# liudabao001/JABD-Joint-Attention-Based-Detector-for-small-face-detection

Hardware: AMD Instinct MI355X
Metric: images/sec at 1024x1024 bs32 (1/2/4/8 GPU); boxes/sec NMS (higher is better)
Workload: dtype fp32; 1 GPU; C2: JABD-MobileNetV3 RetinaFace (nets/retinaface_r.py) eval forward, weights_init weights; global_batch=32, image_size=1024, parallelism=replicas x1

## Files before the change

include/jabd.h:

```cpp
#ifndef JABD_H_
#define JABD_H_

#include <stddef.h>
#include <stdint.h>

#ifdef __cplusplus
extern "C" {
#endif

typedef void* jabd_stream_t;

enum {
  JABD_OK = 0,
  JABD_EINVAL = 1,
  JABD_EHIP = 2,
  JABD_EWS = 3,
};

const char* jabd_version(void);
int64_t jabd_abi_struct_size(int32_t which);
int jabd_last_error(char* buf, size_t len);

int jabd_decode_f32(const float* loc, const float* priors, int64_t batch,
                    int64_t num_priors, float var0, float var1, float* boxes,
// ... 113 lines not shown
                               const int64_t* counts,
                               float* grad_loc, float* grad_conf,
                               float* grad_landm, jabd_stream_t stream);
int jabd_multibox_diou_loss_fwd_f32(const float* loc, const float* conf,
                                    const float* landm, const float* loc_t,
                                    const int64_t* conf_t, const float* landm_t,
                                    const float* priors, float var0, float var1,
                                    int64_t batch, int64_t num_priors, int neg_pos,
                                    float* sums, int64_t* counts, uint8_t* sel,
                                    void* ws, size_t ws_bytes, jabd_stream_t stream);
int jabd_multibox_diou_loss_bwd_f32(const float* loc, const float* conf,
                                    const float* landm, const float* loc_t,
                                    const int64_t* conf_t, const float* landm_t,
                                    const float* priors, float var0, float var1,
                                    const uint8_t* sel, int64_t batch,
                                    int64_t num_priors, const float* gout,
                                    const int64_t* counts, float* grad_loc,
                                    float* grad_conf, float* grad_landm,
                                    jabd_stream_t stream);
int jabd_multibox_loss_finalize_f32(const float* sums, const int64_t* counts,
                                    float* loss, jabd_stream_t stream);

enum {
  JABD_ACT_NONE = 0,
  JABD_ACT_RELU = 1,
  JABD_ACT_LEAKY = 2,
  JABD_ACT_HSWISH = 3,
  JABD_ACT_HSIGMOID = 4,
  JABD_ACT_SIGMOID = 5,
};

typedef struct jabd_conv_args {
  const float* x; int64_t x_bs; int32_t x_ps, x_c0;
  int32_t B, H, W, Cin;
  const float* x2; int64_t x2_bs; int32_t x2_ps, Cin2;
  int32_t x2_W, x2_stride;
  const float* ascale; int64_t ascale_bs;
  const void* w; const float* bias;
  const float* res; int64_t res_bs; int32_t res_ps, res_c0;
  float* y; int64_t y_bs; int32_t y_ps, y_c0;
  int32_t OH, OW, Cout, Ntiles, tn, Kc;
  int32_t KH, KW, stride, pad;
  int32_t act; float slope;
  int32_t nchw_in, tconv;
  int32_t flags, reserved1;
  int64_t M;
  const void* w32; int32_t ntiles32, tn32;
  float* y2; int64_t y2_bs; int32_t y2_ps, y2_c0, nsplit, act2; float slope2; int32_t reserved2;
  void* ws; int64_t ws_bytes;
} jabd_conv_args;
int64_t jabd_conv_workspace_size(const jabd_conv_args* args);
int jabd_conv_pack_tn(int cout);
int jabd_conv_pack_tn32(int cout);
int jabd_conv_pack_f32(const float* w, int32_t cout, int32_t cin, int32_t kh, int32_t kw,
                       int32_t transposed, int32_t Kc, int32_t Ntiles, float* wp, int32_t K8,
                       int32_t NT32, float* wp32, jabd_stream_t stream);
int jabd_conv_pack_multi_f32(const int64_t* jobs, const int64_t* starts, int32_t njobs,
                             int64_t total, jabd_stream_t stream);
int jabd_conv2d_nhwc_f32(const jabd_conv_args* args, jabd_stream_t stream);
int64_t jabd_conv1x1_bn_stats_nblk(const jabd_conv_args* args);
int64_t jabd_conv_bn_bwd_part_floats(const jabd_conv_args* args);
int jabd_conv_bn_bwd_sums_f32(const jabd_conv_args* args, const float* x, int32_t x_ps,
                              const float* mean, const float* invstd, const float* gamma,
                              const float* beta, int32_t act, float slope, float* part,
                              int64_t part_floats, jabd_stream_t stream);
int jabd_conv_bn_bwd_sums_res_f32(const jabd_conv_args* args, const float* x, int32_t x_ps,
                                  const float* mask, int32_t mask_ps, const float* mean,
                                  const float* invstd, float* part, int64_t part_floats,
                                  jabd_stream_t stream);
int jabd_bn_act_bwd_rows_f32(float* part, const float* dy, const float* x, int64_t M,
                             int32_t C, const float* mean, const float* invstd,
                             const float* gamma, const float* beta, int32_t act, float slope,
                             float* dgamma, float* dbeta, float* dx, jabd_stream_t stream);
int64_t jabd_conv_bn_stats_part_floats(const jabd_conv_args* args);
int jabd_conv_bn_stats_f32(const jabd_conv_args* args, float* part, int64_t part_floats,
                           float* mean, float* invstd, float* running_mean, float* running_var,
                           float momentum, float eps, jabd_stream_t stream);
int jabd_conv1x1_bn_stats_f32(const jabd_conv_args* args, float* part, int64_t nblk,
                              float* shift, jabd_stream_t stream);

int jabd_stem_nchw_f32(const float* x, int32_t B, int32_t H, int32_t W, const float* w,
                       const float* bias, int32_t act, float* y, jabd_stream_t stream);

typedef struct jabd_dw_args {
  const float* x; int64_t x_bs; int32_t x_ps, reserved0;
  int32_t B, H, W, C;
  const float* w; const float* bias;
  float* y; int64_t y_bs; int32_t y_ps, reserved1;
  int32_t OH, OW, k, stride, pad, act;
  float slope; int32_t nblk;
  float* part;
} jabd_dw_args;
int64_t jabd_dw_nblk(int64_t B, int64_t OH, int64_t OW, int64_t C);
int jabd_dwconv_nhwc_f32(const jabd_dw_args* args, jabd_stream_t stream);
int64_t jabd_dwconv_stats_nblk(int64_t B, int64_t OH, int64_t OW, int64_t C);
int jabd_dwconv_stats_f32(const jabd_dw_args* args, float* stats_part, float* shift,
                          jabd_stream_t stream);
int jabd_dwconv_bnin_stats_f32(const jabd_dw_args* args, const float* mean, const float* invstd,
                               const float* gamma, const float* beta, int32_t act, float slope,
                               float* stats_part, float* shift, jabd_stream_t stream);

typedef struct jabd_expdw_args {
  const float* x; int64_t x_bs; int32_t x_ps, Cin;
  int32_t B, H, W, E;
  const void* we; const float* be; int32_t Ntiles, Kc;
  const float* wd; const float* bd;
// ... 200 lines not shown
```

jabd-joint-attention-based-detector-for-small-face-detection_amd/csrc/conv32.hip:

```cpp
#include <stdlib.h>

#include <algorithm>

#include "common.h"
#include "conv_args.h"

namespace jabd {

typedef float f32x16 __attribute__((ext_vector_type(16)));

__device__ __forceinline__ float act32(float v, int act, float slope) {
  switch (act) {
    case ACT_RELU: return relu_f(v);
    case ACT_LEAKY: return v > 0.f ? v : v * slope;
    case ACT_HSWISH: return hswish_f(v);
    case ACT_HSIGMOID: return hsigmoid_f(v);
    case ACT_SIGMOID: return 1.f / (1.f + expf(-v));
    default: return v;
  }
}

constexpr int kBK = 32;

__device__ __forceinline__ void wave_lds_sync32() {
  asm volatile("s_waitcnt lgkmcnt(0)" ::: "memory");
  __builtin_amdgcn_wave_barrier();
}
constexpr int kG = kBK / 8;
constexpr int kGateLds = 1024;

constexpr int kEpiPitch = 36;
enum { kEpiRt = 0, kEpiNone = 1, kEpiRes = 2 };
template <int TN, bool ST, bool BB, int EPI = kEpiRt>
__device__ __forceinline__ void m32_epilogue_tm1(const ConvArgs& p, const f32x16 (&acc)[TN],
                                                 int pm, int om, int nb, int srow, float* ep,
                                                 float* __restrict__ part, const BnEpi& bb,
                                                 int lane) {
  const bool has_bias = EPI == kEpiRt && p.bias;
  const bool has_res = EPI == kEpiRes || (EPI == kEpiRt && p.res);
  const int h = lane >> 5, j = lane & 31;
  const int ep_px = lane >> 3, ep_q = lane & 7;
  int mrow[4], prow[4];
#pragma unroll
  for (int r = 0; r < 4; ++r) {
    prow[r] = __shfl(pm, ep_px + 8 * r);
    mrow[r] = __shfl(om, ep_px + 8 * r);
  }
#pragma unroll
  for (int u = 0; u < TN; ++u) {
    const int nb0 = (nb * TN + u) * 32;
    if (nb0 >= p.Cout) break;
    const int n = nb0 + 4 * ep_q;
    float4 ss = make_float4(0.f, 0.f, 0.f, 0.f), sq = ss, sh = ss;
    float4 bmu = sh, bis = sh, bgm = sh, bbt = sh;
    float4 bx[4], bmk[4];
    if constexpr (BB) {
      if (n < p.Cout) {
        bmu = *reinterpret_cast<const float4*>(bb.mean + n);
        bis = *reinterpret_cast<const float4*>(bb.invstd + n);
        if (!bb.mask) {
          bgm = *reinterpret_cast<const float4*>(bb.gamma + n);
          bbt = *reinterpret_cast<const float4*>(bb.beta + n);
        }
      }
#pragma unroll
      for (int r = 0; r < 4; ++r)
        bx[r] = (prow[r] >= 0 && n < p.Cout)
                    ? *reinterpret_cast<const float4*>(bb.x + (int64_t)mrow[r] * bb.x_ps + n)
                    : sh;
      if (bb.mask) {
#pragma unroll
        for (int r = 0; r < 4; ++r)
          bmk[r] = (prow[r] >= 0 && n < p.Cout)
                       ? *reinterpret_cast<const float4*>(bb.mask + (int64_t)mrow[r] * bb.mask_ps + n)
                       : sh;
      }
    }
#pragma unroll
    for (int c = 0; c < 4; ++c)
      *reinterpret_cast<float4*>(ep + j * kEpiPitch + 8 * c + 4 * h) =
          make_float4(acc[u][4 * c], acc[u][4 * c + 1], acc[u][4 * c + 2],
                      acc[u][4 * c + 3]);
    wave_lds_sync32();
    if constexpr (ST) sh = *reinterpret_cast<const float4*>(ep + 4 * ep_q);
#pragma unroll
    for (int r = 0; r < 4; ++r) {
      const int px = ep_px + 8 * r;
      if (prow[r] < 0 || n >= p.Cout) continue;
      float4 v = *reinterpret_cast<const float4*>(ep + px * kEpiPitch + 4 * ep_q);
      if (BB && bb.mask) {
        if (p.res) {
          const float4 rr = *reinterpret_cast<const float4*>(p.res + (int64_t)mrow[r] * p.res_ps +
                                                             p.res_c0 + n);
          v.x += rr.x; v.y += rr.y; v.z += rr.z; v.w += rr.w;
        }
        v.x *= bmk[r].x > 0.f ? 1.f : 0.f;
        v.y *= bmk[r].y > 0.f ? 1.f : 0.f;
        v.z *= bmk[r].z > 0.f ? 1.f : 0.f;
        v.w *= bmk[r].w > 0.f ? 1.f : 0.f;
        const float xh0 = (bx[r].x - bmu.x) * bis.x, xh1 = (bx[r].y - bmu.y) * bis.y;
        const float xh2 = (bx[r].z - bmu.z) * bis.z, xh3 = (bx[r].w - bmu.w) * bis.w;
        ss.x += v.x; ss.y += v.y; ss.z += v.z; ss.w += v.w;
        sq.x += v.x * xh0; sq.y += v.y * xh1; sq.z += v.z * xh2; sq.w += v.w * xh3;
        *reinterpret_cast<float4*>(p.y + (int64_t)mrow[r] * p.y_ps + p.y_c0 + n) = v;
// ... 278 lines not shown
      for (int u = 0; u < TN; ++u) bw[u] = bs[(q * TN + u) * 64 + lane];
#pragma unroll
      for (int t = 0; t < TM; ++t)
#pragma unroll
        for (int u = 0; u < TN; ++u)
          acc[t][u] = __builtin_amdgcn_mfma_f32_32x32x2f32(bw[u].x, a_cur[t][q].x, acc[t][u], 0, 0, 0);
#pragma unroll
      for (int t = 0; t < TM; ++t)
#pragma unroll
        for (int u = 0; u < TN; ++u)
          acc[t][u] = __builtin_amdgcn_mfma_f32_32x32x2f32(bw[u].y, a_cur[t][q].y, acc[t][u], 0, 0, 0);
#pragma unroll
      for (int t = 0; t < TM; ++t)
#pragma unroll
        for (int u = 0; u < TN; ++u)
          acc[t][u] = __builtin_amdgcn_mfma_f32_32x32x2f32(bw[u].z, a_cur[t][q].z, acc[t][u], 0, 0, 0);
#pragma unroll
      for (int t = 0; t < TM; ++t)
#pragma unroll
        for (int u = 0; u < TN; ++u)
          acc[t][u] = __builtin_amdgcn_mfma_f32_32x32x2f32(bw[u].w, a_cur[t][q].w, acc[t][u], 0, 0, 0);
    }
    if (more) {
      store_b((s + 1) & 1, s + 1, b_nxt);
#pragma unroll
      for (int t = 0; t < TM; ++t)
#pragma unroll
        for (int q = 0; q < kG; ++q) a_cur[t][q] = a_nxt[t][q];
    }
    __syncthreads();
  }

  if (ks > 1) {
    const int npad = p.Ntiles * 32;
    float* pb = part + (int64_t)blockIdx.y * p.M * npad;
#pragma unroll
    for (int t = 0; t < TM; ++t) {
      if (pm[t] < 0) continue;
      float* prow = pb + (int64_t)om[t] * npad;
#pragma unroll
      for (int u = 0; u < TN; ++u)
#pragma unroll
        for (int c = 0; c < 4; ++c) {
          const int n = (nb * TN + u) * 32 + 8 * c + 4 * h;
          *reinterpret_cast<float4*>(prow + n) = make_float4(
              acc[t][u][4 * c], acc[t][u][4 * c + 1], acc[t][u][4 * c + 2], acc[t][u][4 * c + 3]);
        }
    }
    return;
  }
  if constexpr (TM == 1) {
    float* ep = reinterpret_cast<float*>(sB_) + wave * 32 * kEpiPitch;
    const int srow = mb * 4 + wave;
    m32_epilogue_tm1<TN, ST, BB, (ST || BB) ? kEpiNone : EPI>(p, acc[0], pm[0], om[0], nb, srow,
                                                                ep, part, bb, lane);
    return;
  }
#pragma unroll
  for (int t = 0; t < TM; ++t) {
    const int m = om[t];
    if (pm[t] < 0) continue;
    float* yrow = p.y + (int64_t)m * p.y_ps + p.y_c0;
    const float* rrow = p.res ? p.res + (int64_t)m * p.res_ps + p.res_c0 : nullptr;
#pragma unroll
    for (int u = 0; u < TN; ++u)
#pragma unroll
      for (int c = 0; c < 4; ++c) {
        const int n = (nb * TN + u) * 32 + 8 * c + 4 * h;
        if (n >= p.Cout) continue;
        float4 v = make_float4(acc[t][u][4 * c], acc[t][u][4 * c + 1], acc[t][u][4 * c + 2],
                               acc[t][u][4 * c + 3]);
        if (p.bias) {
          const float4 bb = *reinterpret_cast<const float4*>(p.bias + n);
          v.x += bb.x; v.y += bb.y; v.z += bb.z; v.w += bb.w;
        }
        if (rrow) {
          const float4 rr = *reinterpret_cast<const float4*>(rrow + n);
          v.x += rr.x; v.y += rr.y; v.z += rr.z; v.w += rr.w;
        }
        v.x = act32(v.x, p.act, p.slope);
        v.y = act32(v.y, p.act, p.slope);
        v.z = act32(v.z, p.act, p.slope);
        v.w = act32(v.w, p.act, p.slope);
        *reinterpret_cast<float4*>(yrow + n) = v;
      }
  }

}

__global__ __launch_bounds__(256) void m32_ksplit_reduce(const ConvArgs p, int ks,
                                                         const float* __restrict__ part) {
  const int npad = p.Ntiles * 32, c4n = (p.Cout + 3) >> 2;
  const int64_t i = blockIdx.x * (int64_t)blockDim.x + threadIdx.x;
  if (i >= p.M * c4n) return;
  const int64_t m = i / c4n;
  const int n = (int)(i - m * c4n) * 4;
  float4 v = *reinterpret_cast<const float4*>(part + m * npad + n);
  for (int y = 1; y < ks; ++y) {
    const float4 q = *reinterpret_cast<const float4*>(part + ((int64_t)y * p.M + m) * npad + n);
    v.x += q.x; v.y += q.y; v.z += q.z; v.w += q.w;
  }
  if (p.bias) {
    const float4 bb = *reinterpret_cast<const float4*>(p.bias + n);
    v.x += bb.x; v.y += bb.y; v.z += bb.z; v.w += bb.w;
  }
  if (p.res) {
    const float4 rr = *reinterpret_cast<const float4*>(p.res + m * p.res_ps + p.res_c0 + n);
    v.x += rr.x; v.y += rr.y; v.z += rr.z; v.w += rr.w;
  }
  v.x = act32(v.x, p.act, p.slope);
  v.y = act32(v.y, p.act, p.slope);
  v.z = act32(v.z, p.act, p.slope);
  v.w = act32(v.w, p.act, p.slope);
  *reinterpret_cast<float4*>(p.y + m * p.y_ps + p.y_c0 + n) = v;
}

template <int TN, int KS, bool ST, bool BB, int EPI>
__global__ __launch_bounds__(256) void conv1x1_m32s_kernel(const ConvArgs p, int nblk_n,
                                                            float* __restrict__ part,
                                                            const BnEpi bb) {
  constexpr int NW4 = KS * kG * TN * 64;
  extern __shared__ __attribute__((aligned(16))) float4 m32s_lds[];
  const int lane = threadIdx.x & 63;
  const int wave = __builtin_amdgcn_readfirstlane(threadIdx.x >> 6);
  const int h = lane >> 5, j = lane & 31;
  const int xcd = blockIdx.x & 7, rr = blockIdx.x >> 3;
  const int nb = rr % nblk_n, wgm = (rr / nblk_n) * 8 + xcd;
  const int gm = gridDim.x / nblk_n;
  {
    const float4* wg = reinterpret_cast<const float4*>(p.w);
    for (int f = threadIdx.x; f < NW4; f += 256) {
      const int k8 = f / (TN * 64), rem = f - k8 * (TN * 64);
      m32s_lds[f] = wg[((int64_t)k8 * p.Ntiles + nb * TN + (rem >> 6)) * 64 + (rem & 63)];
    }
  }
  __syncthreads();
  float* ep = reinterpret_cast<float*>(m32s_lds + NW4) + wave * 32 * kEpiPitch;
  const int64_t ntiles = (p.M + 31) >> 5;
  const int64_t step = (int64_t)gm * 4;
  const float* xb = p.x + p.x_c0 + 4 * h;
  auto load = [&](int64_t T, int s, int q) {
    const int64_t m = T * 32 + j;
    return m < p.M ? *reinterpret_cast<const float4*>(xb + m * p.x_ps + s * kBK + 8 * q)
                   : make_float4(0.f, 0.f, 0.f, 0.f);
  };
  float4 a[KS][kG];
  int64_t T = (int64_t)wgm * 4 + wave;
#pragma unroll
  for (int s = 0; s < KS; ++s)
#pragma unroll
    for (int q = 0; q < kG; ++q) a[s][q] = load(T, s, q);
  for (; T < ntiles; T += step) {
    const int64_t Tn = T + step;
    f32x16 acc[TN];
#pragma unroll
    for (int u = 0; u < TN; ++u)
#pragma unroll
      for (int r = 0; r < 16; ++r) acc[u][r] = 0.f;
#pragma unroll
    for (int s = 0; s < KS; ++s)
#pragma unroll
      for (int q = 0; q < kG; ++q) {
        float4 bw[TN];
#pragma unroll
        for (int u = 0; u < TN; ++u) bw[u] = m32s_lds[((s * kG + q) * TN + u) * 64 + lane];
#pragma unroll
        for (int u = 0; u < TN; ++u)
          acc[u] = __builtin_amdgcn_mfma_f32_32x32x2f32(bw[u].x, a[s][q].x, acc[u], 0, 0, 0);
#pragma unroll
        for (int u = 0; u < TN; ++u)
          acc[u] = __builtin_amdgcn_mfma_f32_32x32x2f32(bw[u].y, a[s][q].y, acc[u], 0, 0, 0);
#pragma unroll
        for (int u = 0; u < TN; ++u)
          acc[u] = __builtin_amdgcn_mfma_f32_32x32x2f32(bw[u].z, a[s][q].z, acc[u], 0, 0, 0);
#pragma unroll
        for (int u = 0; u < TN; ++u)
          acc[u] = __builtin_amdgcn_mfma_f32_32x32x2f32(bw[u].w, a[s][q].w, acc[u], 0, 0, 0);
        a[s][q] = load(Tn, s, q);
      }
    const int64_t m = T * 32 + j;
    const int pm = m < p.M ? (int)m : -1;
    m32_epilogue_tm1<TN, ST, BB, EPI>(p, acc, pm, pm, nb, (int)T, ep, part, bb, lane);
  }
}

static int m32_ksplit(const ConvArgs& a, bool kxk, int64_t grid) {
  if (a.tconv || a.Cout % 4 || grid >= 256) return 1;
  const int Kt = kxk ? a.KH * a.KW * a.Cin : a.Cin + (a.x2 ? a.Cin2 : 0);
  const int S = (Kt + kBK - 1) / kBK;
  int ks = (int)std::min<int64_t>(8, (512 + grid - 1) / grid);
  ks = std::min(ks, S / 4);
  return ks >= 2 ? ks : 1;
}
static int64_t m32_ksplit_bytes(const ConvArgs& a, int ks) {
  return ks > 1 ? (int64_t)ks * a.B * a.OH * a.OW * a.ntiles32 * 32 * (int64_t)sizeof(float) : 0;
}

template <int TM, int TN, bool KXK, bool AS>
static int launch_m32_as(const ConvArgs& a, hipStream_t st);

template <int TM, int TN, bool KXK>
static int launch_m32(const ConvArgs& a, hipStream_t st) {
  if (a.ascale) return launch_m32_as<TM, TN, KXK, true>(a, st);
  return launch_m32_as<TM, TN, KXK, false>(a, st);
}

template <int TM, int TN, bool KXK, bool AS>
static int launch_m32_as(const ConvArgs& a, hipStream_t st) {
  constexpr int BM = 4 * 32 * TM;
  const int64_t OHW = (int64_t)a.OH * a.OW;
  const int per_img = a.ascale != nullptr;
  const int64_t mt_img = cdiv(OHW, BM);
  if (KXK && a.tconv && a.stride == 2) {
    JABD_REQUIRE(!per_img, "conv32: phase mode without ascale");
    for (int ph = 0; ph < 2; ++ph)
      for (int pw = 0; pw < 2; ++pw) {
        const int64_t Mp = (int64_t)a.B * ((a.OH - ph + 1) / 2) * ((a.OW - pw + 1) / 2);
        if (Mp <= 0) continue;
        const int64_t grid = cdiv(Mp, BM) * (a.Ntiles / TN);
        JABD_REQUIRE(grid < (int64_t)0x7fffffff, "conv32: grid too large");
        conv1x1_m32_kernel<TM, TN, KXK, AS><<<(unsigned)grid, 256, 0, st>>>(a, (int)mt_img, 0,
                                                                        2 * ph + pw, 1, nullptr,
                                                                        BnEpi{});
        if (int e = check_launch("conv1x1_m32")) return e;
      }
    return JABD_OK;
  }
  const int64_t mtiles = per_img ? mt_img * a.B : cdiv(a.M, BM);
  const int64_t grid = mtiles * (a.Ntiles / TN);
  JABD_REQUIRE(grid < (int64_t)0x7fffffff, "conv32: grid too large");
  const int ks = a.ws ? m32_ksplit(a, KXK, grid) : 1;
  if (ks > 1 && a.ws_bytes >= m32_ksplit_bytes(a, ks)) {
    float* part = static_cast<float*>(a.ws);
    conv1x1_m32_kernel<TM, TN, KXK, AS><<<dim3((unsigned)grid, (unsigned)ks), 256, 0, st>>>(
        a, (int)mt_img, per_img, -1, ks, part, BnEpi{});
    if (int e = check_launch("conv1x1_m32 (split K)")) return e;
    const int64_t n4 = a.M * ((a.Cout + 3) / 4);
    m32_ksplit_reduce<<<(unsigned)cdiv(n4, 256), 256, 0, st>>>(a, ks, part);
    return check_launch("m32_ksplit_reduce");
  }
  if constexpr (TM == 1 && !AS) {
    if (!a.bias && a.act == ACT_NONE) {
      if (a.res)
        conv1x1_m32_kernel<1, TN, KXK, false, false, false, kEpiRes>
            <<<(unsigned)grid, 256, 0, st>>>(a, (int)mt_img, per_img, -1, 1, nullptr, BnEpi{});
      else
        conv1x1_m32_kernel<1, TN, KXK, false, false, false, kEpiNone>
            <<<(unsigned)grid, 256, 0, st>>>(a, (int)mt_img, per_img, -1, 1, nullptr, BnEpi{});
      return check_launch("conv1x1_m32");
    }
  }
  conv1x1_m32_kernel<TM, TN, KXK, AS><<<(unsigned)grid, 256, 0, st>>>(a, (int)mt_img, per_img, -1,
                                                                     1, nullptr, BnEpi{});
  return check_launch("conv1x1_m32");
}

static bool m32s_on() {
  static const bool on = [] {
    const char* e = getenv("JABD_M32S");
    return !(e && e[0] == '0');
  }();
  return on;
}

// ... 103 lines not shown
using namespace jabd;

static int m32_tm(const ConvArgs& a) {
  static int ftm = -1;
  if (ftm < 0) {
    const char* e = getenv("JABD_M32_TM");
    ftm = e ? atoi(e) : 0;
  }
  if (a.tn32 > 4) return 1;
  if (ftm == 1 || ftm == 2) return ftm;
  return (!a.ascale || a.M < 65536) ? 1 : 2;
}

static int m32_tn_launch(const ConvArgs& a) {
  static const bool off = [] {
    const char* e = getenv("JABD_M32_TN1");
    return e && e[0] == '0';
  }();
  if (off || a.tn32 <= 1 || a.tconv || !a.ascale) return a.tn32;
  const int64_t BM = 4 * 32 * m32_tm(a);
  const int64_t OHW = (int64_t)a.OH * a.OW;
  const int64_t mtiles = a.ascale ? cdiv(OHW, BM) * a.B : cdiv((int64_t)a.B * OHW, BM);
  return mtiles * (a.ntiles32 / a.tn32) >= 256 ? a.tn32 : 1;
}

extern "C" int64_t jabd_conv_workspace_size(const jabd_conv_args* args) {
  if (!args) return 0;
  const ConvArgs& a = *args;
  if (!a.w32 || a.Cin % 32 || a.tconv || a.nchw_in || a.tn32 <= 0) return 0;
  const bool kxk = !(a.KH == 1 && a.KW == 1 && a.stride == 1 && a.pad == 0);
  ConvArgs am = a;
  am.M = (int64_t)a.B * a.OH * a.OW;
  const int tn = m32_tn_launch(am);
  const int TM = tn == a.tn32 ? m32_tm(am) : 1;
  const int64_t BM = 4 * 32 * TM;
  const int64_t OHW = (int64_t)a.OH * a.OW;
  const int64_t mtiles = a.ascale ? cdiv(OHW, BM) * a.B : cdiv((int64_t)a.B * OHW, BM);
  const int64_t grid = mtiles * (a.ntiles32 / tn);
  return m32_ksplit_bytes(a, m32_ksplit(a, kxk, grid));
}

extern "C" int jabd_conv_pack_tn32(int cout) {
  const int nt = (cout + 31) / 32;
  if (nt <= 4) return nt;
  if (nt % 4 == 0) return 4;
  int best = 4, waste = (nt + 3) / 4 * 4 - nt;
  for (int tn : {5, 6, 7}) {
    const int w = (nt + tn - 1) / tn * tn - nt;
    if (w < waste) { waste = w; best = tn; }
  }
  return best;
}

namespace jabd {
int conv1x1_m32_dispatch(const ConvArgs& a0, hipStream_t st, bool kxk) {
  ConvArgs a = a0;
  a.w = a0.w32;
  a.Ntiles = a0.ntiles32;
  if (!kxk) {
    const int r = m32s_dispatch(a, a0.tn32, nullptr, BnEpi{}, 0, st);
    if (r >= 0) return r;
  }
#define M32(TM_, TN_) \
  return kxk ? launch_m32<TM_, TN_, true>(a, st) : launch_m32<TM_, TN_, false>(a, st);
  if (m32_tn_launch(a0) == 1 && a0.tn32 > 1) M32(1, 1)
  if (m32_tm(a0) == 1) {
    switch (a0.tn32) {
      case 1: M32(1, 1)
      case 2: M32(1, 2)
      case 3: M32(1, 3)
      case 4: M32(1, 4)
      default: break;
    }
  }
  switch (a0.tn32) {
    case 1: M32(2, 1)
    case 2: M32(2, 2)
    case 3: M32(2, 3)
    case 4: M32(2, 4)
    case 5: M32(1, 5)
    case 6: M32(1, 6)
    case 7: M32(1, 7)
    default: return -1;
  }
#undef M32
}
}

namespace jabd {

__device__ __forceinline__ float w2d_at(const float* __restrict__ w, int cout, int cin, int khw,
                                        int transposed, int k, int n) {
  const int cinp = transposed ? cout : cin;
  const int ncols = transposed ? cin : cout;
  if (k >= khw * cinp || n >= ncols) return 0.f;
  const int tap = k / cinp, c = k - tap * cinp;
  const int co = transposed ? c : n, ci = transposed ? n : c;
  return w[((int64_t)co * cin + ci) * khw + tap];
}

__global__ __launch_bounds__(256) void pack_w_kernel(const float* __restrict__ w, int cout,
                                                     int cin, int khw, int transposed, int Kc,
                                                     int Ntiles, float* __restrict__ wp, int K8,
                                                     int NT32, float* __restrict__ wp32) {
  const int64_t i = blockIdx.x * (int64_t)blockDim.x + threadIdx.x;
  const int64_t n16 = (int64_t)Kc * Ntiles * 64;
  if (i < n16) {
    const int lane = (int)(i & 63);
    const int64_t r = i >> 6;
    const int nt = (int)(r % Ntiles), kc = (int)(r / Ntiles);
    const int g = lane >> 4, j = lane & 15;
    float4 v;
    v.x = w2d_at(w, cout, cin, khw, transposed, 16 * kc + 4 * g + 0, 16 * nt + j);
    v.y = w2d_at(w, cout, cin, khw, transposed, 16 * kc + 4 * g + 1, 16 * nt + j);
// ... 98 lines not shown
```

jabd-joint-attention-based-detector-for-small-face-detection_amd/jabd_amd/_lib.py:

```python
import ctypes
import os
import threading

import torch

_HERE = os.path.dirname(os.path.abspath(__file__))
LIB_PATH = os.environ.get("JABD_LIB") or os.path.join(_HERE, "libjabd.so")

c_i64 = ctypes.c_int64
c_int = ctypes.c_int
c_f32 = ctypes.c_float
c_f64 = ctypes.c_double
c_size = ctypes.c_size_t
c_vp = ctypes.c_void_p
c_sizep = ctypes.POINTER(ctypes.c_size_t)

c_i32 = ctypes.c_int32
c_fp = ctypes.POINTER(ctypes.c_float)


class ConvArgs(ctypes.Structure):
    _fields_ = [
        ("x", c_vp), ("x_bs", c_i64), ("x_ps", c_i32), ("x_c0", c_i32),
        ("B", c_i32), ("H", c_i32), ("W", c_i32), ("Cin", c_i32),
# ... 80 lines not shown
                              c_vp, c_vp, c_vp, c_vp, c_size, c_vp],
    "jabd_multibox_workspace_size": [c_i64, c_i64, c_sizep],
    "jabd_multibox_loss_fwd_f32": [c_vp, c_vp, c_vp, c_vp, c_vp, c_vp, c_i64, c_i64, c_int,
                                   c_vp, c_vp, c_vp, c_vp, c_size, c_vp],
    "jabd_multibox_loss_bwd_f32": [c_vp, c_vp, c_vp, c_vp, c_vp, c_vp, c_vp, c_i64, c_i64,
                                   c_vp, c_vp, c_vp, c_vp, c_vp, c_vp],
    "jabd_multibox_loss_finalize_f32": [c_vp, c_vp, c_vp, c_vp],
    "jabd_letterbox_f32": [c_vp, c_i64, c_int, c_int, c_vp, c_int, c_int, c_f32, c_vp, c_int,
                           c_vp],
    "jabd_correct_boxes_f32": [c_vp, c_i64, c_int, c_int, c_int, c_int, c_int, c_int, c_vp],
    "jabd_augment_workspace_size": [c_int, c_int, c_sizep],
    "jabd_augment_u8": [c_vp, c_int, c_int, c_int, c_int, c_int, c_int, c_int, c_int, c_int,
                        c_f64, c_f32, c_f32, c_vp, c_vp, c_size, c_vp],
    "jabd_wider_eval_workspace_size": [c_i64, c_i64, c_sizep],
    "jabd_wider_eval_f64": [c_vp, c_vp, c_vp, c_vp, c_vp, c_i64, c_i64, c_i64, c_f64, c_int,
                            c_vp, c_vp, c_size, c_vp],
    "jabd_upsample_bicubic_ac_f32": [c_vp, c_i64, c_int, c_int, c_int, c_vp, c_int, c_int, c_vp],
    "jabd_upsample_bicubic_ac_bwd_f32": [c_vp, c_i64, c_int, c_int, c_int, c_vp, c_int, c_int,
                                         c_vp],
    "jabd_nlm_attn_fwd_f32": [c_vp, c_vp, c_vp, c_i32, c_i32, c_i32, c_i32, c_vp, c_vp, c_vp],
    "jabd_nlm_attn_bwd_f32": [c_vp, c_vp, c_vp, c_vp, c_vp, c_vp, c_i32, c_i32, c_i32, c_i32,
                              c_vp, c_vp, c_vp, c_vp],
    "jabd_window_copy_multi_f32": [c_i32, ctypes.POINTER(WindowCopy), c_vp],
    "jabd_transpose_f32": [c_vp, c_i32, c_i32, c_vp, c_vp],
    "jabd_colsum_f32": [c_vp, c_i64, c_i32, c_vp, c_vp],
    "jabd_sum_multi_f32": [c_i32, ctypes.POINTER(c_vp), c_i64, c_vp, c_vp],
    "jabd_weighted_sum3_f32": [c_vp, c_vp, c_vp, c_f32, c_vp, c_vp],
    "jabd_conv_w2d_f32": [c_vp, c_i32, c_i32, c_i32, c_vp, c_vp],
    "jabd_heads_wpack_f32": [c_vp, c_vp, c_vp, c_vp, c_vp, c_vp, c_i32, c_i32, c_i32, c_i32,
                             c_vp, c_i32, c_vp, c_i32, c_vp],
    "jabd_nlm_attn_dkv_ws_floats": [c_i32, c_i32, c_i32, c_i32],
    "jabd_nlm_attn_dkv_f32": [c_vp, c_vp, c_vp, c_vp, c_i32, c_i32, c_i32, c_i32, c_vp, c_i64,
                              c_vp, c_vp, c_vp],
    "jabd_add3_f32": [c_vp, c_vp, c_vp, c_i64, c_vp, c_vp],
    "jabd_beca_ws_floats": [c_i64, c_i64, c_int],
    "jabd_conv_pack_multi_f32": [c_vp, c_vp, c_i32, c_i64, c_vp],
    "jabd_ssh_tail_weight_floats": [],
    "jabd_ssh_tail_heads_f32": [c_vp, c_i64, c_i32, c_vp, c_i64, c_i32, c_i32, c_i32, c_vp, c_f32,
                                c_i64, c_i64, c_i32, c_vp, c_vp, c_vp, c_vp],
    "jabd_conv_pack_f32": [c_vp, c_i32, c_i32, c_i32, c_i32, c_i32, c_i32, c_i32, c_vp, c_i32,
                           c_i32, c_vp, c_vp],
    "jabd_beca_fwd_f32": [c_vp, c_i64, c_i64, c_int, c_vp, c_int, c_vp, c_vp, c_vp, c_i64, c_vp],
    "jabd_beca_bwd_f32": [c_vp, c_vp, c_i64, c_i64, c_int, c_vp, c_int, c_vp, c_vp, c_vp, c_vp,
                          c_vp, c_i64, c_vp],
    "jabd_match_iou_f32": [c_vp, c_vp, c_i64, c_i64, c_vp, c_i64, c_f32, c_f32, c_f32,
                           c_vp, c_vp, c_vp, c_vp, c_size, c_vp],
    "jabd_multibox_diou_loss_fwd_f32": [c_vp, c_vp, c_vp, c_vp, c_vp, c_vp, c_vp, c_f32, c_f32,
                                        c_i64, c_i64, c_int, c_vp, c_vp, c_vp, c_vp, c_size,
                                        c_vp],
    "jabd_multibox_diou_loss_bwd_f32": [c_vp, c_vp, c_vp, c_vp, c_vp, c_vp, c_vp, c_f32, c_f32,
                                        c_vp, c_i64, c_i64, c_vp, c_vp, c_vp, c_vp, c_vp, c_vp],
    "jabd_conv_pack_tn": [c_int],
    "jabd_conv_pack_tn32": [c_int],
    "jabd_conv2d_nhwc_f32": [ctypes.POINTER(ConvArgs), c_vp],
    "jabd_conv1x1_bn_stats_nblk": [ctypes.POINTER(ConvArgs)],
    "jabd_conv1x1_bn_stats_f32": [ctypes.POINTER(ConvArgs), c_vp, c_i64, c_vp, c_vp],
    "jabd_conv_workspace_size": [ctypes.POINTER(ConvArgs)],
    "jabd_conv_bn_stats_part_floats": [ctypes.POINTER(ConvArgs)],
    "jabd_conv_bn_bwd_part_floats": [ctypes.POINTER(ConvArgs)],
    "jabd_conv_bn_bwd_sums_f32": [ctypes.POINTER(ConvArgs), c_vp, c_i32, c_vp, c_vp, c_vp, c_vp,
                                  c_i32, c_f32, c_vp, c_i64, c_vp],
    "jabd_conv_bn_bwd_sums_res_f32": [ctypes.POINTER(ConvArgs), c_vp, c_i32, c_vp, c_i32, c_vp,
                                      c_vp, c_vp, c_i64, c_vp],
    "jabd_bn_act_bwd_rows_f32": [c_vp, c_vp, c_vp, c_i64, c_i32, c_vp, c_vp, c_vp, c_vp, c_i32,
                                 c_f32, c_vp, c_vp, c_vp, c_vp],
    "jabd_conv_bn_stats_f32": [ctypes.POINTER(ConvArgs), c_vp, c_i64, c_vp, c_vp, c_vp, c_vp,
                               c_f32, c_f32, c_vp],
    "jabd_stem_nchw_f32": [c_vp, c_i32, c_i32, c_i32, c_vp, c_vp, c_i32, c_vp, c_vp],
    "jabd_dw_nblk": [c_i64, c_i64, c_i64, c_i64],
    "jabd_dwconv_nhwc_f32": [ctypes.POINTER(DwArgs), c_vp],
    "jabd_dwconv_stats_nblk": [c_i64, c_i64, c_i64, c_i64],
    "jabd_dwconv_stats_f32": [ctypes.POINTER(DwArgs), c_vp, c_vp, c_vp],
    "jabd_dwconv_bnin_stats_f32": [ctypes.POINTER(DwArgs), c_vp, c_vp, c_vp, c_vp, c_i32, c_f32,
                                   c_vp, c_vp, c_vp],
    "jabd_bn_stats_final_f32": [c_vp, c_vp, c_i64, c_i64, c_i32, c_vp, c_vp, c_vp, c_vp, c_f32,
                                c_f32, c_vp],
    "jabd_expand_dw_nblk": [c_i32, c_i32, c_i32, c_i32],
    "jabd_expand_dw_nhwc_f32": [ctypes.POINTER(ExpDwArgs), c_vp],
    "jabd_expand_dw_select": [c_i32],
    "jabd_channel_sum_f32": [c_vp, c_i64, c_i32, c_i64, c_i64, c_i64, c_i64, c_vp, c_vp],
    "jabd_partial_reduce_f32": [c_vp, c_i64, c_i64, c_i64, c_i64, c_vp, c_vp],
    "jabd_eca_gate_f32": [c_vp, c_i64, c_i64, c_i64, c_i64, c_vp, c_i32, c_i32, c_vp, c_vp,
                          c_vp],
    "jabd_nlm_pool_f32": [c_vp, c_i64, c_i32, c_i32, c_i32, c_i32, c_i32, c_i32, c_i32, c_vp,
                          c_vp, c_vp, c_vp, c_i32, ctypes.POINTER(c_i32), c_i32, c_vp, c_vp,
                          c_vp, c_vp],
    "jabd_nlm_apply_f32": [c_vp, c_i64, c_i32, c_i32, c_i32, c_i32, c_i32, c_i32, c_i32, c_vp,
                           c_vp, c_vp, c_vp, c_i32, c_i32, c_vp, c_vp, c_vp, c_vp, c_vp, c_vp,
                           c_vp],
    "jabd_maxpool_nhwc_f32": [c_vp, c_i32, c_i32, c_i32, c_i32, c_i32, c_i32, c_i32, c_vp, c_vp],
    "jabd_heads_scatter_f32": [c_vp, c_i32, c_i64, c_i64, c_i64, c_i32, c_vp, c_vp, c_vp, c_vp],
    "jabd_heads_f32": [c_vp, c_i64, c_i32, c_i32, c_i32, c_i32, c_vp, c_vp, c_i64, c_i64, c_i32,
                       c_vp, c_vp, c_vp, c_vp],
    "jabd_bn_nblk": [c_i64, c_i32],
    "jabd_bn_stats_f32": [c_vp, c_i32, c_i64, c_i32, c_vp, c_vp, c_vp, c_vp, c_vp, c_f32, c_f32,
                          c_vp],
    "jabd_bn_act_fwd_f32": [c_vp, c_i32, c_i64, c_i32, c_vp, c_vp, c_vp, c_vp, c_vp, c_i32,
                            c_i32, c_f32, c_vp, c_i32, c_i32, c_vp],
    "jabd_bn_act_bwd_f32": [c_vp, c_i32, c_i32, c_vp, c_i32, c_vp, c_i32, c_i64, c_i32, c_vp,
                            c_vp, c_vp, c_vp, c_i32, c_f32, c_vp, c_vp, c_vp, c_vp, c_vp, c_vp],
    "jabd_conv_wgrad_part_floats": [ctypes.POINTER(ConvArgs)],
    "jabd_conv_wgrad_f32": [ctypes.POINTER(ConvArgs), c_vp, c_vp, c_vp],
    "jabd_eca_pool_gate_multi_f32": [c_i32, c_i64, c_vp, c_vp, c_vp, c_vp, c_vp, c_vp, c_vp, c_vp,
                                     c_vp, c_i32, c_vp, c_vp],
    "jabd_bn_sum_nblk": [c_i64, c_i32],
    "jabd_bn_act_fwd_sum_f32": [c_vp, c_i64, c_i32, c_vp, c_vp, c_vp, c_vp, c_i32, c_f32, c_vp,
# ... 110 lines not shown
```

Before: 5024 images/sec.

## Add 8-wave 1x1 conv kernel splitting N tiles across wave groups for small grids

Adds a 512-thread variant of the gated 1x1 MFMA conv in which two groups of four waves each take half of the N tiles of a block. It shares the double-buffered weight tile and the LDS-staged gate scale between the groups. The variant is used only when a per-image activation scale is present, no k-split applies, and the 4-wave grid would be smaller than twice the CU count. The aim is to give more waves per CU on small late-stage feature maps, at the cost of more register and LDS pressure per block. An environment variable and an API call let the user force 4 or 8 waves, and another call reports which path ran last.

```diff
diff --git a/include/jabd.h b/include/jabd.h
--- a/include/jabd.h
+++ b/include/jabd.h
@@ -189,6 +189,8 @@
 int64_t jabd_conv_workspace_size(const jabd_conv_args* args);
 int jabd_conv_pack_tn(int cout);
 int jabd_conv_pack_tn32(int cout);
+int jabd_conv_m32_nw_select(int32_t nw);
+int jabd_conv_m32_nw_last(void);
 int jabd_conv_pack_f32(const float* w, int32_t cout, int32_t cin, int32_t kh, int32_t kw,
                        int32_t transposed, int32_t Kc, int32_t Ntiles, float* wp, int32_t K8,
                        int32_t NT32, float* wp32, jabd_stream_t stream);
diff --git a/jabd-joint-attention-based-detector-for-small-face-detection_amd/csrc/conv32.hip b/jabd-joint-attention-based-detector-for-small-face-detection_amd/csrc/conv32.hip
--- a/jabd-joint-attention-based-detector-for-small-face-detection_amd/csrc/conv32.hip
+++ b/jabd-joint-attention-based-detector-for-small-face-detection_amd/csrc/conv32.hip
@@ -33,9 +33,9 @@
 enum { kEpiRt = 0, kEpiNone = 1, kEpiRes = 2 };
 template <int TN, bool ST, bool BB, int EPI = kEpiRt>
 __device__ __forceinline__ void m32_epilogue_tm1(const ConvArgs& p, const f32x16 (&acc)[TN],
-                                                 int pm, int om, int nb, int srow, float* ep,
+                                                 int pm, int om, int nt0, int srow, float* ep,
                                                  float* __restrict__ part, const BnEpi& bb,
-                                                 int lane) {
+                                                 int lane, int ntn = TN) {
   const bool has_bias = EPI == kEpiRt && p.bias;
   const bool has_res = EPI == kEpiRes || (EPI == kEpiRt && p.res);
   const int h = lane >> 5, j = lane & 31;
@@ -48,8 +48,8 @@
   }
 #pragma unroll
   for (int u = 0; u < TN; ++u) {
-    const int nb0 = (nb * TN + u) * 32;
-    if (nb0 >= p.Cout) break;
+    const int nb0 = (nt0 + u) * 32;
+    if (u >= ntn || nb0 >= p.Cout) break;
     const int n = nb0 + 4 * ep_q;
     float4 ss = make_float4(0.f, 0.f, 0.f, 0.f), sq = ss, sh = ss;
     float4 bmu = sh, bis = sh, bgm = sh, bbt = sh;
@@ -434,7 +434,7 @@
   if constexpr (TM == 1) {
     float* ep = reinterpret_cast<float*>(sB_) + wave * 32 * kEpiPitch;
     const int srow = mb * 4 + wave;
-    m32_epilogue_tm1<TN, ST, BB, (ST || BB) ? kEpiNone : EPI>(p, acc[0], pm[0], om[0], nb, srow,
+    m32_epilogue_tm1<TN, ST, BB, (ST || BB) ? kEpiNone : EPI>(p, acc[0], pm[0], om[0], nb * TN, srow,
                                                                 ep, part, bb, lane);
     return;
   }
@@ -470,6 +470,154 @@
 
 }
 
+template <int TN>
+__global__ __launch_bounds__(512) void conv1x1_m32w8_kernel(const ConvArgs p, int mtiles_img) {
+  constexpr int BM = 4 * 32;
+  constexpr int TN0 = (TN + 1) / 2;
+  constexpr int NB4 = kG * TN * 64;
+  constexpr int NBT = (NB4 + 511) / 512;
+  constexpr int kEpi4 = 8 * 32 * kEpiPitch / 4;
+  constexpr int SB4 = kEpi4 > 2 * NB4 ? kEpi4 : 2 * NB4;
+  static_assert(TN >= 2, "two N groups");
+  __shared__ float4 sB_[SB4];
+  float4 (*sB)[NB4] = reinterpret_cast<float4 (*)[NB4]>(sB_);
+  __shared__ __attribute__((aligned(16))) float sGate[kGateLds];
+  const int lane = threadIdx.x & 63;
+  const int wave = __builtin_amdgcn_readfirstlane(threadIdx.x >> 6);
+  const int wm = wave & 3, ng = wave >> 2;
+  const int u0 = ng * TN0;
+  const int nu = ng ? TN - TN0 : TN0;
+  const int h = lane >> 5, j = lane & 31;
+  const int nblk_n = p.Ntiles / TN;
+  const int bid = blockIdx.x;
+  const int nb = bid % nblk_n, mb = bid / nblk_n;
+  const int OHW = p.OH * p.OW;
+  const int img = mb / mtiles_img;
+  const int m_lo = img * OHW + (mb - img * mtiles_img) * BM;
+  const int m_hi = min(img * OHW + OHW, (int)p.M);
+  const int m = m_lo + wm * 32 + j;
+  const int pm = m < m_hi ? m : -1;
+  const int Kt = p.Cin + (p.x2 ? p.Cin2 : 0);
+  const int S = (Kt + kBK - 1) / kBK;
+  const int x2_pix = (p.x2 && p.x2_stride != 1) ? (int)(p.x2_bs / p.x2_ps) : 0;
+  const float4* wg = reinterpret_cast<const float4*>(p.w);
+  const float* sc = p.ascale + (int64_t)img * p.ascale_bs;
+  const bool gate_lds = p.Cin <= kGateLds;
+
+  auto load_a = [&](int s, float4 (&a)[kG]) {
+#pragma unroll
+    for (int q = 0; q < kG; ++q) {
+      const int k4 = s * kBK + 8 * q + 4 * h;
+      float4 r = make_float4(0.f, 0.f, 0.f, 0.f);
+      if (pm >= 0) {
+        if (k4 < p.Cin) {
+          r = *reinterpret_cast<const float4*>(p.x + (int64_t)pm * p.x_ps + p.x_c0 + k4);
+        } else if (k4 < Kt) {
+          int qq = pm;
+          if (p.x2_stride != 1) {
+            const int b = pm / OHW, rr = pm - b * OHW;
+            const int oh = rr / p.OW, ow = rr - oh * p.OW;
+            qq = b * x2_pix + (oh * p.x2_stride) * p.x2_W + ow * p.x2_stride;
+          }
+          r = *reinterpret_cast<const float4*>(p.x2 + (int64_t)qq * p.x2_ps + (k4 - p.Cin));
+        }
+      }
+      a[q] = r;
+    }
+  };
+  auto load_b = [&](int s, float4 (&b)[NBT]) {
+#pragma unroll
+    for (int i = 0; i < NBT; ++i) {
+      const int f = i * 512 + threadIdx.x;
+      float4 v = make_float4(0.f, 0.f, 0.f, 0.f);
+      if (f < NB4) {
+        const int g = f / (TN * 64), rem = f - g * (TN * 64);
+        const int u = rem >> 6, l = rem & 63;
+        const int k8 = s * kG + g;
+        v = wg[((int64_t)k8 * p.Ntiles + nb * TN + u) * 64 + l];
+        if (!gate_lds) {
+          const int k0 = 8 * k8 + 4 * (l >> 5);
+          if (k0 < p.Cin) {
+            const float4 s4 = *reinterpret_cast<const float4*>(sc + k0);
+            v.x *= s4.x; v.y *= s4.y; v.z *= s4.z; v.w *= s4.w;
+          }
+        }
+      }
+      b[i] = v;
+    }
+  };
+  auto store_b = [&](int buf, int s, const float4 (&b)[NBT]) {
+#pragma unroll
+    for (int i = 0; i < NBT; ++i) {
+      const int f = i * 512 + threadIdx.x;
+      if (f < NB4) {
+        float4 v = b[i];
+        if (gate_lds) {
+          const int g = f / (TN * 64), l = f & 63;
+          const int k0 = 8 * (s * kG + g) + 4 * (l >> 5);
+          if (k0 < p.Cin) {
+            const float4 s4 = *reinterpret_cast<const float4*>(sGate + k0);
+            v.x *= s4.x; v.y *= s4.y; v.z *= s4.z; v.w *= s4.w;
+          }
+        }
+        sB[buf][f] = v;
+      }
+    }
+  };
+
+  f32x16 acc[TN0];
+#pragma unroll
+  for (int u = 0; u < TN0; ++u)
+#pragma unroll
+    for (int r = 0; r < 16; ++r) acc[u][r] = 0.f;
+
+  float4 a_cur[kG], a_nxt[kG], b_nxt[NBT];
+  if (gate_lds) {
+    for (int i = threadIdx.x; i < p.Cin; i += 512) sGate[i] = sc[i];
+    __syncthreads();
+  }
+  load_a(0, a_cur);
+  load_b(0, b_nxt);
+  store_b(0, 0, b_nxt);
+  __syncthreads();
+  for (int s = 0; s < S; ++s) {
+    const bool more = s + 1 < S;
+    if (more) {
+      load_a(s + 1, a_nxt);
+      load_b(s + 1, b_nxt);
+    }
+    const float4* bs = sB[s & 1] + u0 * 64 + lane;
+#pragma unroll
+    for (int q = 0; q < kG; ++q) {
+      float4 bw[TN0];
+#pragma unroll
+      for (int u = 0; u < TN0; ++u)
+        if (u + 1 < TN0 || TN % 2 == 0 || u < nu) bw[u] = bs[(q * TN + u) * 64];
+#pragma unroll
+      for (int e = 0; e < 4; ++e)
+#pragma unroll
+        for (int u = 0; u < TN0; ++u)
+          if (u + 1 < TN0 || TN % 2 == 0 || u < nu) {
+            const float bv = e == 0 ? bw[u].x : e == 1 ? bw[u].y : e == 2 ? bw[u].z : bw[u].w;
+            const float av = e == 0   ? a_cur[q].x
+                             : e == 1 ? a_cur[q].y
+                             : e == 2 ? a_cur[q].z
+                                      : a_cur[q].w;
+            acc[u] = __builtin_amdgcn_mfma_f32_32x32x2f32(bv, av, acc[u], 0, 0, 0);
+          }
+    }
+    if (more) {
+      store_b((s + 1) & 1, s + 1, b_nxt);
+#pragma unroll
+      for (int q = 0; q < kG; ++q) a_cur[q] = a_nxt[q];
+    }
+    __syncthreads();
+  }
+  float* ep = reinterpret_cast<float*>(sB_) + wave * 32 * kEpiPitch;
+  m32_epilogue_tm1<TN0, false, false, kEpiRt>(p, acc, pm, pm, nb * TN + u0, 0, ep, nullptr,
+                                              BnEpi{}, lane, nu);
+}
+
 __global__ __launch_bounds__(256) void m32_ksplit_reduce(const ConvArgs p, int ks,
                                                          const float* __restrict__ part) {
   const int npad = p.Ntiles * 32, c4n = (p.Cout + 3) >> 2;
@@ -562,7 +710,7 @@
       }
     const int64_t m = T * 32 + j;
     const int pm = m < p.M ? (int)m : -1;
-    m32_epilogue_tm1<TN, ST, BB, EPI>(p, acc, pm, pm, nb, (int)T, ep, part, bb, lane);
+    m32_epilogue_tm1<TN, ST, BB, EPI>(p, acc, pm, pm, nb * TN, (int)T, ep, part, bb, lane);
   }
 }
 
@@ -578,6 +726,8 @@
   return ks > 1 ? (int64_t)ks * a.B * a.OH * a.OW * a.ntiles32 * 32 * (int64_t)sizeof(float) : 0;
 }
 
+static int m32_nw_last = 0;
+
 template <int TM, int TN, bool KXK, bool AS>
 static int launch_m32_as(const ConvArgs& a, hipStream_t st);
 
@@ -592,6 +742,7 @@
   constexpr int BM = 4 * 32 * TM;
   const int64_t OHW = (int64_t)a.OH * a.OW;
   const int per_img = a.ascale != nullptr;
+  m32_nw_last = 4;
   const int64_t mt_img = cdiv(OHW, BM);
   if (KXK && a.tconv && a.stride == 2) {
     JABD_REQUIRE(!per_img, "conv32: phase mode without ascale");
@@ -801,6 +952,62 @@
   return best;
 }
 
+static int m32_nw_force = 0;
+static int m32_nw_sel() {
+  static const int env = [] {
+    const char* e = getenv("JABD_M32_NW");
+    return e && e[0] == '8' ? 8 : (e && e[0] == '4' ? 4 : 0);
+  }();
+  return m32_nw_force ? m32_nw_force : env;
+}
+
+extern "C" int jabd_conv_m32_nw_select(int32_t nw) {
+  const int prev = m32_nw_force;
+  m32_nw_force = nw == 4 || nw == 8 ? nw : 0;
+  return prev;
+}
+
+extern "C" int jabd_conv_m32_nw_last(void) { return m32_nw_last; }
+
+template <int TN>
+static int launch_m32w8(const ConvArgs& a, hipStream_t st) {
+  const int64_t mt_img = cdiv((int64_t)a.OH * a.OW, (int64_t)128);
+  const int64_t grid = mt_img * a.B * (a.Ntiles / TN);
+  JABD_REQUIRE(grid < (int64_t)0x7fffffff && a.M < ((int64_t)1 << 31) - 128,
+               "conv32: grid too large");
+  conv1x1_m32w8_kernel<TN><<<(unsigned)grid, 512, 0, st>>>(a, (int)mt_img);
+  m32_nw_last = 8;
+  return check_launch("conv1x1_m32 (8 waves)");
+}
+
+static int m32w8_dispatch(const ConvArgs& a, hipStream_t st) {
+  const int sel = m32_nw_sel();
+  if (sel == 4 || !a.ascale || a.tconv || a.tn32 < 2 || a.tn32 > 7 || a.Ntiles % a.tn32) return -1;
+  const int64_t OHW = (int64_t)a.OH * a.OW;
+  const int tn = m32_tn_launch(a);
+  const int TM = tn == a.tn32 ? m32_tm(a) : 1;
+  const int64_t grid4 = cdiv(OHW, (int64_t)128 * TM) * a.B * (a.ntiles32 / tn);
+  if (a.ws && m32_ksplit(a, false, grid4) > 1) return -1;
+  if (sel != 8) {
+    static int ncu = 0;
+    if (!ncu) {
+      int dev = 0;
+      JABD_HIP(hipGetDevice(&dev));
+      JABD_HIP(hipDeviceGetAttribute(&ncu, hipDeviceAttributeMultiprocessorCount, dev));
+    }
+    if (tn != a.tn32 || TM != 1 || grid4 >= 2 * (int64_t)ncu) return -1;
+  }
+  switch (a.tn32) {
+    case 2: return launch_m32w8<2>(a, st);
+    case 3: return launch_m32w8<3>(a, st);
+    case 4: return launch_m32w8<4>(a, st);
+    case 5: return launch_m32w8<5>(a, st);
+    case 6: return launch_m32w8<6>(a, st);
+    case 7: return launch_m32w8<7>(a, st);
+    default: return -1;
+  }
+}
+
 namespace jabd {
 int conv1x1_m32_dispatch(const ConvArgs& a0, hipStream_t st, bool kxk) {
   ConvArgs a = a0;
@@ -809,6 +1016,8 @@
   if (!kxk) {
     const int r = m32s_dispatch(a, a0.tn32, nullptr, BnEpi{}, 0, st);
     if (r >= 0) return r;
+    const int r8 = m32w8_dispatch(a, st);
+    if (r8 >= 0) return r8;
   }
 #define M32(TM_, TN_) \
   return kxk ? launch_m32<TM_, TN_, true>(a, st) : launch_m32<TM_, TN_, false>(a, st);
diff --git a/jabd-joint-attention-based-detector-for-small-face-detection_amd/jabd_amd/_lib.py b/jabd-joint-attention-based-detector-for-small-face-detection_amd/jabd_amd/_lib.py
--- a/jabd-joint-attention-based-detector-for-small-face-detection_amd/jabd_amd/_lib.py
+++ b/jabd-joint-attention-based-detector-for-small-face-detection_amd/jabd_amd/_lib.py
@@ -156,6 +156,8 @@
                                         c_vp, c_i64, c_i64, c_vp, c_vp, c_vp, c_vp, c_vp, c_vp],
     "jabd_conv_pack_tn": [c_int],
     "jabd_conv_pack_tn32": [c_int],
+    "jabd_conv_m32_nw_select": [c_i32],
+    "jabd_conv_m32_nw_last": [],
     "jabd_conv2d_nhwc_f32": [ctypes.POINTER(ConvArgs), c_vp],
     "jabd_conv1x1_bn_stats_nblk": [ctypes.POINTER(ConvArgs)],
     "jabd_conv1x1_bn_stats_f32": [ctypes.POINTER(ConvArgs), c_vp, c_i64, c_vp, c_vp],
```

New measurement: 5063 images/sec, median of 6. No clear change (+0.8%).
